# vishal-2000/EDMP

Measured on AMD Instinct MI355X. Metric: guided denoise-steps/sec (trajectories x reverse steps), higher is better.
Workload: dtype f32

## Files before the change

### edmp_amd/csrc/bf3.hip

```cpp
#pragma once
#include <type_traits>

#include "params.h"
#include "wide.hip"

namespace edmp {

constexpr int kBf3Threads = 512;

typedef __attribute__((ext_vector_type(8))) __bf16 bf16x8_t;
typedef __attribute__((ext_vector_type(2))) __bf16 bf16x2_t;
typedef __attribute__((ext_vector_type(4))) float f32x4_t;
typedef __attribute__((ext_vector_type(4))) unsigned u32x4_t;
typedef __attribute__((ext_vector_type(2))) unsigned u32x2_t;

inline unsigned short bf16_rne_bits(float x) {
    unsigned u = __builtin_bit_cast(unsigned, x);
    u += 0x7fffu + ((u >> 16) & 1u);
    return (unsigned short)(u >> 16);
}
inline float bf16_bits_to_float(unsigned short b) { return __builtin_bit_cast(float, (unsigned)b << 16); }
inline void split3_bf16_rne(float x, unsigned short (&c)[3]) {
    c[0] = bf16_rne_bits(x);
    const float r1 = x - bf16_bits_to_float(c[0]);
    c[1] = bf16_rne_bits(r1);
    const float r2 = r1 - bf16_bits_to_float(c[1]);
    c[2] = bf16_rne_bits(r2);
}

template <int KIND, int MS, int CG, int GS, int LIN, bool RES>
struct Bf3Cfg {
    static constexpr int NTH = kBf3Threads, NMW = 4;
    static constexpr int LOUT = (KIND == WK_K5) ? LIN : (KIND == WK_DOWN) ? (LIN - 1) / 2 + 1 : ((2 * LIN == 8 || 2 * LIN == 14 || 2 * LIN == 26) ? 2 * LIN - 1 : 2 * LIN);
    static constexpr bool GN = (KIND == WK_K5);
    static constexpr int SW = 16, S = CG / SW, PARTS = NMW / S;
    static constexpr bool ROWSPLIT = (PARTS == 2 && MS == 32);
    static constexpr int NR = (PARTS == 1) ? MS / 16 : 1;
    static constexpr bool RES_ONE_ACC = RES && MS == 16 && LIN >= 13;
    static constexpr int KC = 32;
    static constexpr int RS = KC + 8;
    static constexpr int PLANE = MS * RS;
    static constexpr int STAGE = LIN * 3 * PLANE;
    static constexpr int NTAP = (KIND == WK_K5) ? 5 : (KIND == WK_DOWN) ? 3 : 4;
    static constexpr int NSLOT = NTAP + (RES ? 1 : 0);
    static constexpr int WBLK = NSLOT * 3 * 1024;
    static constexpr int slot(int l, int lp) {
        const int t = (KIND == WK_K5) ? lp - l + 2 : (KIND == WK_DOWN) ? lp - 2 * l + 1 : l + 1 - 2 * lp;
        return (t >= 0 && t < NTAP) ? t : -1;
    }
    static constexpr int NTILE = LOUT + (RES ? LIN : 0);
    static constexpr int tslot(int tile, int lp) { return tile < LOUT ? slot(tile, lp) : (tile - LOUT == lp ? NTAP : -1); }
    static constexpr int pairs_of(int l) {
        int n = (RES && l < LIN) ? 1 : 0;
        for (int lp = 0; lp < LIN; ++lp) n += slot(l, lp) >= 0 ? 1 : 0;
        return n;
    }
    static constexpr int total_pairs() {
        int n = 0;
        for (int l = 0; l < LOUT; ++l) n += pairs_of(l);
        return n;
    }
    static constexpr unsigned part0_mask() {
        if (ROWSPLIT || PARTS == 1) return ~0u;
        const int tot = total_pairs();
        int pc[16] = {};
        for (int l = 0; l < LOUT; ++l) pc[l] = pairs_of(l);
        unsigned best = 0;
        int bestmax = 1 << 30;
        for (unsigned m = 1; m < (1u << LOUT) - 1; m += 2) {
            int n = 0;
            for (int l = 0; l < LOUT; ++l) n += ((m >> l) & 1u) ? pc[l] : 0;
            const int mx = n > tot - n ? n : tot - n;
            if (mx < bestmax) bestmax = mx, best = m;
        }
        return best;
    }
    static constexpr unsigned P0 = part0_mask();
    static constexpr bool owned(int tile, int H) {
        if (ROWSPLIT || PARTS == 1) return true;
        const int l = tile < LOUT ? tile : tile - LOUT;
        return (int)((P0 >> l) & 1u) == (H == 0 ? 1 : 0);
    }
    static constexpr int local(int tile, int H) {
        int n = 0;
        for (int q = 0; q < tile; ++q) n += owned(q, H) ? 1 : 0;
        return n;
    }
    static constexpr int ntiles(int H) { return local(NTILE, H); }
    static constexpr int MAXT = ntiles(0) > ntiles(1) ? ntiles(0) : ntiles(1);
    static constexpr bool needed(int H, int lp) {
        for (int t = 0; t < NTILE; ++t)
            if (owned(t, H) && tslot(t, lp) >= 0) return true;
        return false;
    }
    static constexpr int ord(int H, int q) {
        int n = 0;
        for (int i = 0; i < q; ++i) n += needed(H, i % LIN) ? 1 : 0;
        return n;
    }
    static constexpr int next(int H, int q) {
        for (int i = q + 1; i < 2 * LIN; ++i)
            if (needed(H, i % LIN)) return i;
        return -1;
    }
    static constexpr int first(int H) { return needed(H, 0) ? 0 : next(H, 0); }
    static constexpr int A_F4 = LIN * MS * (KC / 4);
    static constexpr int NA = (A_F4 + 255) / 256;
    static constexpr int YS = LOUT * CG + 4, RYS = LIN * CG + 4;
    static constexpr int PPR = NTH / MS, ROW_F4 = LOUT * CG / 4, NF4 = (ROW_F4 + PPR - 1) / PPR;
    static constexpr int RROW_F4 = LIN * CG / 4, RNF4 = (RROW_F4 + PPR - 1) / PPR;
    static constexpr size_t lds_bytes() {
        const size_t a = 2 * (size_t)STAGE * 2, y = (size_t)MS * (YS + (RES ? RYS : 0)) * 4;
        return a > y ? a : y;
    }
    static_assert((CG == 32 && S == 2 && PARTS == 2) || (CG == 64 && S == 4 && PARTS == 1 && MS == 32), "two 16-channel slabs x two parts, or four slabs = the four MFMA waves");
    static_assert(MS == 32 || MS == 16, "32 samples (sample-half parts) or 16 samples (position-set parts)");
    static_assert(!RES || KIND == WK_K5, "the folded residual 1x1 conv belongs to a Conv1dBlock");
    static_assert(!GN || CG % GS == 0, "whole GroupNorm groups per workgroup");
    static_assert((4 * PPR) % CG == 0, "a thread's columns of the final pass lie in one GroupNorm group");
    static_assert(LOUT <= 16, "part0_mask searches 2^LOUT subsets");
};

#ifdef EDMP_BF3_STAMPS
__device__ long long g_bf3_stamps[8][8];
#define EDMP_BF3_STAMP(i) \
    if (blockIdx.x == 0 && lane == 0) g_bf3_stamps[wave][i] = clock64();
#else
#define EDMP_BF3_STAMP(i)
#endif

template <int KIND, int MS, int CG, int GS, int LIN, bool RES>
__global__ __launch_bounds__(kBf3Threads) void bf3_conv_kernel(const float* a_src1, const float* a_src2, const void* a_W, int a_C1, int a_C2, int a_Cout, int a_B,
                                                       int a_gx_shift, int a_ng_shift, RcbP p) {
    using Cf = Bf3Cfg<KIND, MS, CG, GS, LIN, RES>;
    constexpr int LOUT = Cf::LOUT, KC = Cf::KC, RS = Cf::RS, PLANE = Cf::PLANE, STAGE = Cf::STAGE, NSLOT = Cf::NSLOT, NTILE = Cf::NTILE, MAXT = Cf::MAXT;
    constexpr int YS = Cf::YS, RYS = Cf::RYS, NA = Cf::NA, A_F4 = Cf::A_F4, WBLK = Cf::WBLK;
    constexpr bool GN = Cf::GN;
    extern __shared__ __attribute__((aligned(16))) unsigned char lds_raw[];
    unsigned short* stg = reinterpret_cast<unsigned short*>(lds_raw);
    const int tid = threadIdx.x;
    const int lane = tid & 63;
    const int wave = __builtin_amdgcn_readfirstlane(tid >> 6);
    const bool mfma_wave = wave < 4;
    const int s = wave & (Cf::S - 1), part = (Cf::PARTS == 2) ? (wave >> 1) & 1 : 0;
    constexpr int NR = Cf::NR;
    int grp, tile;
    {
        const int lin = blockIdx.x;
        if (a_gx_shift >= 0) {
            const int xcd = lin & 7, j = lin >> 3, ngp_shift = a_ng_shift - a_gx_shift;
            grp = ((j & ((1 << ngp_shift) - 1)) << a_gx_shift) + (xcd & ((1 << a_gx_shift) - 1));
            tile = ((j >> ngp_shift) << (3 - a_gx_shift)) + (xcd >> a_gx_shift);
        } else {
            const int ng = a_Cout / CG;
            grp = lin % ng;
            tile = lin / ng;
        }
    }
    const int co0 = grp * CG, b0 = tile * MS;
    const int ch1 = a_C1 / KC, ch2 = a_C2 / KC, nK = ch1 + ch2;
    EDMP_BF3_STAMP(0)
    asm volatile("v_mov_b32 v255, 0" ::: "v255");

    const int ptid = tid & 255;
    unsigned a_g[NA];
    int a_l[NA];
#pragma unroll
    for (int k = 0; k < NA; ++k) {
        const int e = min(ptid + k * 256, A_F4 - 1);
        const int lp = e / (MS * 8), rem = e % (MS * 8);
        const int row = rem >> 3, quad = rem & 7;
        const int sb = min(b0 + row, a_B - 1);
        a_g[k] = 4u * (unsigned)(((sb - b0) * LIN + lp) * a_C1 + 4 * quad);
        a_l[k] = lp * 3 * PLANE + row * RS + 4 * quad;
    }
    auto fetch = [&](int nc, f32x4(&x)[NA]) __attribute__((always_inline)) {
        const bool first = nc < ch1;
        const char* srcb = reinterpret_cast<const char*>((first ? a_src1 + (size_t)b0 * LIN * a_C1 : a_src2 + (size_t)b0 * LIN * a_C2) + (first ? nc : nc - ch1) * KC);
#pragma unroll
        for (int k = 0; k < NA; ++k) x[k] = *reinterpret_cast<const f32x4*>(srcb + a_g[k]);
    };
    auto commit = [&](unsigned short* st, const f32x4(&x)[NA]) __attribute__((always_inline)) {
#pragma unroll
        for (int k = 0; k < NA; ++k) {
            if ((A_F4 % 256 == 0) || ptid + k * 256 < A_F4) {
                f32x2_t lo2 = {x[k].x, x[k].y}, hi2 = {x[k].z, x[k].w};
#pragma unroll
                for (int m = 0; m < 3; ++m) {
                    const bf16x2_t c01 = __builtin_convertvector(lo2, bf16x2_t), c23 = __builtin_convertvector(hi2, bf16x2_t);
                    *reinterpret_cast<u32x2_t*>(st + a_l[k] + m * PLANE) = u32x2_t{__builtin_bit_cast(unsigned, c01), __builtin_bit_cast(unsigned, c23)};
                    if (m < 2) {
                        lo2 = lo2 - __builtin_convertvector(c01, f32x2_t);
                        hi2 = hi2 - __builtin_convertvector(c23, f32x2_t);
                    }
                }
            }
        }
    };

    const unsigned char* wb = reinterpret_cast<const unsigned char*>(a_W) + ((size_t)(grp * Cf::S + s) * nK) * WBLK + 16 * lane;
    u32x4_t bw[3][NSLOT];
    auto load_w = [&](int kg, auto mc) __attribute__((always_inline)) {
        constexpr int m = decltype(mc)::value;
        const unsigned char* w = wb + (size_t)kg * WBLK + m * 1024;
#pragma unroll
        for (int j = 0; j < NSLOT; ++j) bw[m][j] = *reinterpret_cast<const u32x4_t*>(w + j * 3 * 1024);
    };
    f32x4_t big[MAXT][NR], sml[MAXT][NR];
#pragma unroll
    for (int a = 0; a < MAXT; ++a)
#pragma unroll
        for (int r = 0; r < NR; ++r) {
            big[a][r] = f32x4_t{0.f, 0.f, 0.f, 0.f};
            sml[a][r] = f32x4_t{0.f, 0.f, 0.f, 0.f};
        }
    const int afrag = ((Cf::ROWSPLIT ? 16 * part : 0) + (lane & 15)) * RS + 8 * (lane >> 4);
    constexpr int RBLK = 16 * RS;

    auto chunk = [&](auto hc, const unsigned short* st, int kgn) __attribute__((always_inline)) {
        constexpr int H = decltype(hc)::value;
        u32x4_t av[2][NR][3];
        {
            constexpr int lp0 = Cf::first(H) % LIN;
#pragma unroll
            for (int r = 0; r < NR; ++r) {
                av[0][r][0] = *reinterpret_cast<const u32x4_t*>(st + (lp0 * 3 + 0) * PLANE + r * RBLK + afrag);
                av[0][r][1] = *reinterpret_cast<const u32x4_t*>(st + (lp0 * 3 + 1) * PLANE + r * RBLK + afrag);
            }
        }
        static_for<0, 2>([&](auto pc) __attribute__((always_inline)) {
            constexpr int ph = decltype(pc)::value;
            static_for<0, LIN>([&](auto lpc) __attribute__((always_inline)) {
                constexpr int lp = decltype(lpc)::value;
                constexpr int q = ph * LIN + lp;
                if constexpr (Cf::needed(H, lp)) {
                    constexpr int buf = Cf::ord(H, q) & 1;
                    constexpr int qn = Cf::next(H, q);
                    if constexpr (qn >= 0) {
                        constexpr int lpn = qn % LIN, ncomp = (qn / LIN == 0) ? 2 : 3;
#pragma unroll
                        for (int r = 0; r < NR; ++r)
#pragma unroll
                            for (int m = 0; m < ncomp; ++m) av[buf ^ 1][r][m] = *reinterpret_cast<const u32x4_t*>(st + (lpn * 3 + m) * PLANE + r * RBLK + afrag);
                    }
                    static_for<0, 3>([&](auto kc) __attribute__((always_inline)) {
                        constexpr int k = decltype(kc)::value;
                        constexpr int ia = (ph == 0) ? (k == 1 ? 1 : 0) : 2 - k;
                        constexpr int wc = (ph == 0) ? (k == 0 ? 2 : 1) : 0;
                        static_for<0, NTILE>([&](auto tc) __attribute__((always_inline)) {
                            constexpr int tl = decltype(tc)::value;
                            if constexpr (Cf::owned(tl, H) && Cf::tslot(tl, lp) >= 0) {
                                constexpr int sl = Cf::tslot(tl, lp) >= 0 ? Cf::tslot(tl, lp) : 0;
                                constexpr int la = Cf::local(tl, H);
                                constexpr bool one_acc = Cf::RES_ONE_ACC && tl >= LOUT;
#pragma unroll
                                for (int r = 0; r < NR; ++r) {
                                    if constexpr ((ia == 0 && wc == 0) || one_acc)
                                        big[la][r] = __builtin_amdgcn_mfma_f32_16x16x32_bf16(__builtin_bit_cast(bf16x8_t, av[buf][r][ia]), __builtin_bit_cast(bf16x8_t, bw[wc][sl]), big[la][r], 0, 0, 0);
                                    else
                                        sml[la][r] = __builtin_amdgcn_mfma_f32_16x16x32_bf16(__builtin_bit_cast(bf16x8_t, av[buf][r][ia]), __builtin_bit_cast(bf16x8_t, bw[wc][sl]), sml[la][r], 0, 0, 0);
                                }
                            }
                        });
                    });
                    __builtin_amdgcn_sched_barrier(0);
                }
            });
            if constexpr (ph == 0) {
                load_w(kgn, std::integral_constant<int, 2>{});
                load_w(kgn, std::integral_constant<int, 1>{});
            } else {
                load_w(kgn, std::integral_constant<int, 0>{});
            }
            __builtin_amdgcn_sched_barrier(0);
        });
    };

    f32x4 xa[NA], xb[NA];
    if (!mfma_wave) {
        fetch(0, xa);
        fetch(min(1, nK - 1), xb);
        commit(stg, xa);
        fetch(min(2, nK - 1), xa);
    } else {
        load_w(0, std::integral_constant<int, 2>{});
        load_w(0, std::integral_constant<int, 1>{});
        load_w(0, std::integral_constant<int, 0>{});
    }
    __syncthreads();
    EDMP_BF3_STAMP(1)

    auto mfma_loop = [&](auto hc) __attribute__((always_inline)) {
        for (int c = 0; c < nK; ++c) {
            chunk(hc, stg + (c & 1) * STAGE, min(c + 1, nK - 1));
            __syncthreads();
        }
    };
    if (mfma_wave) {
        if (Cf::ROWSPLIT || Cf::PARTS == 1 || part == 0) mfma_loop(std::integral_constant<int, 0>{});
        else mfma_loop(std::integral_constant<int, 1>{});
    } else {
        for (int c = 0; c < nK; c += 2) {
            if (c + 1 < nK) commit(stg + STAGE, xb);
            if (c + 3 < nK) fetch(c + 3, xb);
            __syncthreads();
            if (c + 1 < nK) {
                if (c + 2 < nK) commit(stg, xa);
                if (c + 4 < nK) fetch(c + 4, xa);
                __syncthreads();
            }
        }
    }
    EDMP_BF3_STAMP(2)

    float* Y = reinterpret_cast<float*>(lds_raw);
    float* R = Y + MS * YS;
    constexpr int PPR = Cf::PPR, ROW_F4 = Cf::ROW_F4, NF4 = Cf::NF4;
    const int erow = tid / PPR, epart = tid % PPR;
    const int eb = min(b0 + erow, a_B - 1);
    float4 g4[GN ? NF4 : 1], be4[GN ? NF4 : 1], ad4[GN ? NF4 : 1];
    if constexpr (GN) {
#pragma unroll
        for (int i = 0; i < NF4; ++i) {
            const int f = min(epart + PPR * i, ROW_F4 - 1);
            const int col = 4 * f;
            const int l = col / CG, ch = co0 + col % CG;
            g4[i] = *reinterpret_cast<const float4*>(p.gamma + ch);
            be4[i] = *reinterpret_cast<const float4*>(p.beta + ch);
            ad4[i] = make_float4(0.f, 0.f, 0.f, 0.f);
            if (p.add_res) ad4[i] = *reinterpret_cast<const float4*>(p.add_res + ((size_t)eb * LOUT + l) * a_Cout + ch);
            else if (p.add_tb) ad4[i] = *reinterpret_cast<const float4*>(p.add_tb + ch);
        }
    }
    auto spill = [&](auto hc) __attribute__((always_inline)) {
        constexpr int H = decltype(hc)::value;
        const int col = s * 16 + (lane & 15);
        const float bias_v = p.bias[co0 + col];
        float rbias_v = 0.f;
        if constexpr (RES) rbias_v = p.res_bias[co0 + col];
        const int row0 = (Cf::ROWSPLIT ? 16 * part : 0) + 4 * (lane >> 4);
        static_for<0, NTILE>([&](auto tc) __attribute__((always_inline)) {
            constexpr int tl = decltype(tc)::value;
            if constexpr (Cf::owned(tl, H)) {
                constexpr int la = Cf::local(tl, H);
#pragma unroll
                for (int rb = 0; rb < NR; ++rb) {
                    if constexpr (tl < LOUT) {
#pragma unroll
                        for (int r = 0; r < 4; ++r) Y[(row0 + 16 * rb + r) * YS + tl * CG + col] = (big[la][rb][r] + sml[la][rb][r]) + bias_v;
                    } else {
#pragma unroll
                        for (int r = 0; r < 4; ++r) R[(row0 + 16 * rb + r) * RYS + (tl - LOUT) * CG + col] = (big[la][rb][r] + sml[la][rb][r]) + rbias_v;
                    }
                }
            }
        });
    };
    if (mfma_wave) {
        if (Cf::ROWSPLIT || Cf::PARTS == 1 || part == 0) spill(std::integral_constant<int, 0>{});
        else spill(std::integral_constant<int, 1>{});
    }
    __syncthreads();
    EDMP_BF3_STAMP(3)
    const int b = b0 + erow;
    if constexpr (RES) {
        if (b < a_B) {
#pragma unroll
            for (int i = 0; i < Cf::RNF4; ++i) {
                const int f = epart + PPR * i;
                if ((Cf::RROW_F4 % PPR == 0) || f < Cf::RROW_F4) {
                    const int col = 4 * f;
                    const int l = col / CG, ch = co0 + col % CG;
                    *reinterpret_cast<float4*>(p.res_out + ((size_t)b * LIN + l) * a_Cout + ch) = *reinterpret_cast<const float4*>(R + erow * RYS + col);
                }
            }
        }
    }
    {
        float4 v[NF4];
        float sum = 0.f;
#pragma unroll
        for (int i = 0; i < NF4; ++i) {
            const int f = epart + PPR * i;
            v[i] = make_float4(0.f, 0.f, 0.f, 0.f);
            if ((ROW_F4 % PPR == 0) || f < ROW_F4) {
                v[i] = *reinterpret_cast<const float4*>(Y + erow * YS + 4 * f);
                sum += (v[i].x + v[i].y) + (v[i].z + v[i].w);
            }
        }
        if constexpr (GN) {
            auto row_group_sum = [&](float x) __attribute__((always_inline)) {
                static_for<0, 4>([&](auto bc) __attribute__((always_inline)) {
                    constexpr int m = 1 << decltype(bc)::value;
                    if constexpr (m < PPR && (GS == CG || (4 * m) % CG < GS)) x = dpp_xor_add<m>(x);
                });
                if constexpr (PPR > 16) x = swap16_add(x);
                static_assert(PPR <= 32, "a sample row's threads lie in one 32-lane half of a wave");
                return x;
            };
            constexpr float inv_n = 1.0f / (float)(LOUT * GS);
            const float mean = row_group_sum(sum) * inv_n;
            float sq = 0.f;
#pragma unroll
            for (int i = 0; i < NF4; ++i) {
                const int f = epart + PPR * i;
                if ((ROW_F4 % PPR == 0) || f < ROW_F4) {
                    const float dx = v[i].x - mean, dy = v[i].y - mean, dz = v[i].z - mean, dw = v[i].w - mean;
                    sq += (dx * dx + dy * dy) + (dz * dz + dw * dw);
                }
            }
            const float rstd = 1.0f / sqrtf(row_group_sum(sq) * inv_n + 1e-5f);
            if (b < a_B) {
#pragma unroll
                for (int i = 0; i < NF4; ++i) {
                    const int f = epart + PPR * i;
                    if ((ROW_F4 % PPR == 0) || f < ROW_F4) {
                        const int col = 4 * f;
                        const int l = col / CG, ch = co0 + col % CG;
                        const float s0 = rstd * g4[i].x, s1 = rstd * g4[i].y, s2 = rstd * g4[i].z, s3 = rstd * g4[i].w;
                        const f32x2_t sa = {s0, s1}, sb = {s2, s3};
                        const f32x2_t ya = mish_fast2(f32x2_t{v[i].x, v[i].y} * sa + (f32x2_t{be4[i].x, be4[i].y} - sa * mean)) + f32x2_t{ad4[i].x, ad4[i].y};
                        const f32x2_t yb = mish_fast2(f32x2_t{v[i].z, v[i].w} * sb + (f32x2_t{be4[i].z, be4[i].w} - sb * mean)) + f32x2_t{ad4[i].z, ad4[i].w};
                        float4 o;
                        o.x = ya.x, o.y = ya.y, o.z = yb.x, o.w = yb.y;
                        *reinterpret_cast<float4*>(p.dst + ((size_t)b * LOUT + l) * a_Cout + ch) = o;
                    }
                }
            }
        } else if (b < a_B) {
#pragma unroll
            for (int i = 0; i < NF4; ++i) {
                const int f = epart + PPR * i;
                if ((ROW_F4 % PPR == 0) || f < ROW_F4) {
                    const int col = 4 * f;
                    const int l = col / CG, ch = co0 + col % CG;
                    *reinterpret_cast<float4*>(p.dst + ((size_t)b * LOUT + l) * a_Cout + ch) = v[i];
                }
            }
        }
    }
    EDMP_BF3_STAMP(4)
}

inline size_t bf3_stream_elems(int cout, int cin, int nslot) { return (size_t)(cout / 16) * (cin / 32) * nslot * 3 * 512; }
inline void pack_fragments_bf3(const float* w_tco_ci, int cout, int cin, int ntap, bool res, unsigned short* out) {
    const size_t n = (size_t)cout * cin;
    const int nkg = cin / 32, nslot = ntap + (res ? 1 : 0);
    for (int sl = 0; sl < cout / 16; ++sl)
        for (int kg = 0; kg < nkg; ++kg)
            for (int slot = 0; slot < nslot; ++slot) {
                const int tap = slot < ntap ? slot : 5;
                for (int lane = 0; lane < 64; ++lane) {
                    const int nn = lane % 16, oct = lane / 16;
                    for (int j = 0; j < 8; ++j) {
                        const float wv = w_tco_ci[(size_t)tap * n + (size_t)(sl * 16 + nn) * cin + 32 * kg + 8 * oct + j];
                        unsigned short c3[3];
                        split3_bf16_rne(wv, c3);
                        for (int comp = 0; comp < 3; ++comp) out[((((size_t)sl * nkg + kg) * nslot + slot) * 3 + comp) * 512 + lane * 8 + j] = c3[comp];
                    }
                }
            }
}

template <int KIND, int MS, int CG, int GS, int LIN, bool RES>
int launch_bf3_t(const RcbP& p, hipStream_t s, KernelAttrs* q) {
    using Cf = Bf3Cfg<KIND, MS, CG, GS, LIN, RES>;
    static std::atomic<int> attr_set{0};
    constexpr size_t bytes = Cf::lds_bytes();
    static_assert(bytes <= 160 * 1024, "bf16x3 position-tile kernel exceeds the 160 KiB LDS of a CU");
    const void* fn = reinterpret_cast<const void*>(&bf3_conv_kernel<KIND, MS, CG, GS, LIN, RES>);
    if (!attr_set.load(std::memory_order_acquire)) {
        EDMP_HIP_CHECK(hipFuncSetAttribute(fn, hipFuncAttributeMaxDynamicSharedMemorySize, (int)bytes));
        attr_set.store(1, std::memory_order_release);
    }
    if (q) {
        hipFuncAttributes fa{};
        EDMP_HIP_CHECK(hipFuncGetAttributes(&fa, fn));
        int wg = 0;
        EDMP_HIP_CHECK(hipOccupancyMaxActiveBlocksPerMultiprocessor(&wg, fn, kBf3Threads, bytes));
        q->regs = fa.numRegs;
        q->block = kBf3Threads;
        q->lds = (int)bytes;
        q->wg_per_cu = wg;
        return EDMP_OK;
    }
    EDMP_REQUIRE(p.C1 % Cf::KC == 0 && p.C2 % Cf::KC == 0 && p.Cout % CG == 0, "bf3_conv_kernel: channels must be multiples of 32 (C1=%d, C2=%d, Cout=%d)", p.C1, p.C2, p.Cout);
    EDMP_REQUIRE(p.C2 == 0 || p.C2 == p.C1, "bf3_conv_kernel: the two halves of a concatenated input must have the same width (C1=%d, C2=%d)", p.C1, p.C2);
    const int ng = p.Cout / CG, nt = (p.B + MS - 1) / MS;
    const int gx = xcd_split(ng, nt, (double)p.Cout * (p.C1 + p.C2) * Cf::NSLOT * 1.5, (double)nt * MS * LIN * (p.C1 + p.C2));
    int gxs = -1, ngs = -1;
    if (gx > 0 && (ng & (ng - 1)) == 0) {
        gxs = __builtin_ctz(gx);
        ngs = __builtin_ctz(ng);
    }
    hipLaunchKernelGGL((bf3_conv_kernel<KIND, MS, CG, GS, LIN, RES>), dim3(ng * nt), dim3(kBf3Threads), bytes, s, p.src1, p.src2, reinterpret_cast<const void*>(p.W), p.C1, p.C2, p.Cout, p.B, gxs, ngs, p);
    return EDMP_OK;
}

}
```

Baseline: 1.150 million.

## Rotate next chunk's first A-fragment read and weight load across the chunk barrier

When the register budget allows (ROTATE), the MFMA waves move the per-chunk barrier inside the chunk, just before the last MFMA group. They then issue the next chunk's first LDS A-fragment reads and its m=0 weight load, so those latencies overlap the tail MFMAs instead of stalling at the start of each chunk. Bias loads are hoisted into the prologue, or before the epilogue when not rotating. Optional cycle counters for barrier time are added under the stamps macro. This raises register pressure, which the KREGS gate is meant to bound.

```diff
diff --git a/edmp_amd/csrc/bf3.hip b/edmp_amd/csrc/bf3.hip
--- a/edmp_amd/csrc/bf3.hip
+++ b/edmp_amd/csrc/bf3.hip
@@ -104,6 +104,8 @@
         return -1;
     }
     static constexpr int first(int H) { return needed(H, 0) ? 0 : next(H, 0); }
+    static constexpr int KREGS = MAXT * NR * 8 + 3 * NSLOT * 4 + 2 * NR * 3 * 4;
+    static constexpr bool ROTATE = KREGS <= 240, BIAS_EARLY = ROTATE;
     static constexpr int A_F4 = LIN * MS * (KC / 4);
     static constexpr int NA = (A_F4 + 255) / 256;
     static constexpr int YS = LOUT * CG + 4, RYS = LIN * CG + 4;
@@ -125,8 +127,15 @@
 __device__ long long g_bf3_stamps[8][8];
 #define EDMP_BF3_STAMP(i) \
     if (blockIdx.x == 0 && lane == 0) g_bf3_stamps[wave][i] = clock64();
+#define EDMP_BF3_CHUNK_BARRIER \
+    bar_t0 = clock64();        \
+    __syncthreads();           \
+    bar_t1 = clock64();
+#define EDMP_BF3_BAR_ADD bar_cyc += bar_t1 - bar_t0;
 #else
 #define EDMP_BF3_STAMP(i)
+#define EDMP_BF3_CHUNK_BARRIER __syncthreads();
+#define EDMP_BF3_BAR_ADD
 #endif
 
 template <int KIND, int MS, int CG, int GS, int LIN, bool RES>
@@ -160,6 +169,9 @@
     const int co0 = grp * CG, b0 = tile * MS;
     const int ch1 = a_C1 / KC, ch2 = a_C2 / KC, nK = ch1 + ch2;
     EDMP_BF3_STAMP(0)
+#ifdef EDMP_BF3_STAMPS
+    long long bar_cyc = 0, bar_t0 = 0, bar_t1 = 0;
+#endif
     asm volatile("v_mov_b32 v255, 0" ::: "v255");
 
     const int ptid = tid & 255;
@@ -217,17 +229,18 @@
     const int afrag = ((Cf::ROWSPLIT ? 16 * part : 0) + (lane & 15)) * RS + 8 * (lane >> 4);
     constexpr int RBLK = 16 * RS;
 
-    auto chunk = [&](auto hc, const unsigned short* st, int kgn) __attribute__((always_inline)) {
+    using AFrag = u32x4_t[2][NR][3];
+    auto read_first = [&](auto hc, AFrag& av, const unsigned short* st) __attribute__((always_inline)) {
+        constexpr int lp0 = Cf::first(decltype(hc)::value) % LIN;
+#pragma unroll
+        for (int r = 0; r < NR; ++r) {
+            av[0][r][0] = *reinterpret_cast<const u32x4_t*>(st + (lp0 * 3 + 0) * PLANE + r * RBLK + afrag);
+            av[0][r][1] = *reinterpret_cast<const u32x4_t*>(st + (lp0 * 3 + 1) * PLANE + r * RBLK + afrag);
+        }
+    };
+    auto chunk = [&](auto hc, AFrag& av, const unsigned short* st, const unsigned short* stn, int kgn, bool more) __attribute__((always_inline)) {
         constexpr int H = decltype(hc)::value;
-        u32x4_t av[2][NR][3];
-        {
-            constexpr int lp0 = Cf::first(H) % LIN;
-#pragma unroll
-            for (int r = 0; r < NR; ++r) {
-                av[0][r][0] = *reinterpret_cast<const u32x4_t*>(st + (lp0 * 3 + 0) * PLANE + r * RBLK + afrag);
-                av[0][r][1] = *reinterpret_cast<const u32x4_t*>(st + (lp0 * 3 + 1) * PLANE + r * RBLK + afrag);
-            }
-        }
+        if constexpr (!Cf::ROTATE) read_first(hc, av, st);
         static_for<0, 2>([&](auto pc) __attribute__((always_inline)) {
             constexpr int ph = decltype(pc)::value;
             static_for<0, LIN>([&](auto lpc) __attribute__((always_inline)) {
@@ -242,6 +255,12 @@
                         for (int r = 0; r < NR; ++r)
 #pragma unroll
                             for (int m = 0; m < ncomp; ++m) av[buf ^ 1][r][m] = *reinterpret_cast<const u32x4_t*>(st + (lpn * 3 + m) * PLANE + r * RBLK + afrag);
+                        if constexpr (Cf::ROTATE && Cf::next(H, qn) < 0) __builtin_amdgcn_sched_barrier(0);
+                    }
+                    if constexpr (qn < 0 && Cf::ROTATE) {
+                        static_assert(ph == 1 && buf == 1, "an even number of entries per chunk: the next chunk's first entry lands in register set 0");
+                        EDMP_BF3_CHUNK_BARRIER
+                        if (more) read_first(hc, av, stn);
                     }
                     static_for<0, 3>([&](auto kc) __attribute__((always_inline)) {
                         constexpr int k = decltype(kc)::value;
@@ -264,19 +283,27 @@
                         });
                     });
                     __builtin_amdgcn_sched_barrier(0);
+                    if constexpr (qn < 0 && Cf::ROTATE) {
+                        EDMP_BF3_BAR_ADD
+                    }
                 }
             });
             if constexpr (ph == 0) {
                 load_w(kgn, std::integral_constant<int, 2>{});
                 load_w(kgn, std::integral_constant<int, 1>{});
-            } else {
+            } else if constexpr (!Cf::ROTATE) {
                 load_w(kgn, std::integral_constant<int, 0>{});
             }
             __builtin_amdgcn_sched_barrier(0);
         });
+        if constexpr (!Cf::ROTATE) {
+            EDMP_BF3_CHUNK_BARRIER
+            EDMP_BF3_BAR_ADD
+        }
     };
 
     f32x4 xa[NA], xb[NA];
+    float bias_v = 0.f, rbias_v = 0.f;
     if (!mfma_wave) {
         fetch(0, xa);
         fetch(min(1, nK - 1), xb);
@@ -285,15 +312,24 @@
     } else {
         load_w(0, std::integral_constant<int, 2>{});
         load_w(0, std::integral_constant<int, 1>{});
-        load_w(0, std::integral_constant<int, 0>{});
+        if constexpr (!Cf::ROTATE) load_w(0, std::integral_constant<int, 0>{});
+        if constexpr (Cf::BIAS_EARLY) {
+            bias_v = p.bias[co0 + s * 16 + (lane & 15)];
+            if constexpr (RES) rbias_v = p.res_bias[co0 + s * 16 + (lane & 15)];
+        }
     }
     __syncthreads();
     EDMP_BF3_STAMP(1)
 
     auto mfma_loop = [&](auto hc) __attribute__((always_inline)) {
+        AFrag av;
+        if constexpr (Cf::ROTATE) read_first(hc, av, stg);
         for (int c = 0; c < nK; ++c) {
-            chunk(hc, stg + (c & 1) * STAGE, min(c + 1, nK - 1));
-            __syncthreads();
+            if constexpr (Cf::ROTATE) {
+                load_w(c, std::integral_constant<int, 0>{});
+                __builtin_amdgcn_sched_barrier(0);
+            }
+            chunk(hc, av, stg + (c & 1) * STAGE, stg + ((c + 1) & 1) * STAGE, min(c + 1, nK - 1), c + 1 < nK);
         }
     };
     if (mfma_wave) {
@@ -303,14 +339,21 @@
         for (int c = 0; c < nK; c += 2) {
             if (c + 1 < nK) commit(stg + STAGE, xb);
             if (c + 3 < nK) fetch(c + 3, xb);
-            __syncthreads();
+            {
+                EDMP_BF3_CHUNK_BARRIER
+                EDMP_BF3_BAR_ADD
+            }
             if (c + 1 < nK) {
                 if (c + 2 < nK) commit(stg, xa);
                 if (c + 4 < nK) fetch(c + 4, xa);
-                __syncthreads();
-            }
-        }
-    }
+                EDMP_BF3_CHUNK_BARRIER
+                EDMP_BF3_BAR_ADD
+            }
+        }
+    }
+#ifdef EDMP_BF3_STAMPS
+    if (blockIdx.x == 0 && lane == 0) g_bf3_stamps[wave][5] = bar_cyc;
+#endif
     EDMP_BF3_STAMP(2)
 
     float* Y = reinterpret_cast<float*>(lds_raw);
@@ -318,6 +361,13 @@
     constexpr int PPR = Cf::PPR, ROW_F4 = Cf::ROW_F4, NF4 = Cf::NF4;
     const int erow = tid / PPR, epart = tid % PPR;
     const int eb = min(b0 + erow, a_B - 1);
+    if constexpr (!Cf::BIAS_EARLY) {
+        if (mfma_wave) {
+            bias_v = p.bias[co0 + s * 16 + (lane & 15)];
+            if constexpr (RES) rbias_v = p.res_bias[co0 + s * 16 + (lane & 15)];
+        }
+        __builtin_amdgcn_sched_barrier(0);
+    }
     float4 g4[GN ? NF4 : 1], be4[GN ? NF4 : 1], ad4[GN ? NF4 : 1];
     if constexpr (GN) {
 #pragma unroll
@@ -335,9 +385,6 @@
     auto spill = [&](auto hc) __attribute__((always_inline)) {
         constexpr int H = decltype(hc)::value;
         const int col = s * 16 + (lane & 15);
-        const float bias_v = p.bias[co0 + col];
-        float rbias_v = 0.f;
-        if constexpr (RES) rbias_v = p.res_bias[co0 + col];
         const int row0 = (Cf::ROWSPLIT ? 16 * part : 0) + 4 * (lane >> 4);
         static_for<0, NTILE>([&](auto tc) __attribute__((always_inline)) {
             constexpr int tl = decltype(tc)::value;
```

After: 1.163 million (median of 6 runs). +1.1%, better.
